# cvg/nice-slam

Measured on NVIDIA H100. Metric: rendered rays/sec, higher is better.
Workload: dtype f32

## Files before the change

nice_slam_b200/csrc/nsb_aux.cu:

```cuda
#include <cstdarg>
#include <cstdio>
#include <cstring>
#include <type_traits>
#include <cuda_fp16.h>
#include "nsb_common.cuh"
#include "nsb_seeds.cuh"
#include "nsb_geom.cuh"

namespace nsb {

static thread_local char g_err[512] = "";
void set_error(const char* fmt, ...) {
  va_list ap; va_start(ap, fmt); vsnprintf(g_err, sizeof(g_err), fmt, ap); va_end(ap);
}
int check_cuda(cudaError_t e, const char* what) {
  if (e == cudaSuccess) return NSB_OK;
  set_error("%s: %s", what, cudaGetErrorString(e));
  (void)cudaGetLastError();
  return NSB_ERR_CUDA;
}

struct PackArgs { nsb_decoder_params p[4]; float* packed[4]; float* flat[4]; int present[4]; };
__device__ __forceinline__ bool pk_mine(int& e) { return (e++ % (int)gridDim.y) == (int)blockIdx.y; }
constexpr int kPackSlices = 32;
// ... 56 lines not shown
    const float h = __uint_as_float(__float_as_uint(v) & 0xffffe000u);
    const int o = ((r >> 3) * (KW >> 2) + (k >> 2)) * 32 + (r & 7) * 4 + (k & 3);
    hi[o] = h; lo[o] = v - h;
  }
}
template <int LV>
__device__ void pack_operands_level(float* __restrict__ img , int& e) {
  using D = Dec<LV>;
  const float* W = img;
  constexpr int PH = D::PH;
  const int o_wh[5] = {0, D::o_W1, D::o_W2, D::o_W3H, D::o_W4};
  float* dst = img + op_fwd_offset(LV);
  if (pk_mine(e)) for (int i = threadIdx.x; i < kHdrFloats; i += blockDim.x) {
    float v = 0.0f;
    if (i < 160) v = W[D::o_b + i];
    else if (i < 320) v = D::XYZ ? W[D::o_bc + (i - 160)] : 0.0f;
    else if (i < 324) v = W[D::o_bo + (i - 320)];
    else if (i >= 336 && i < 464) v = W[D::o_WO + ((i - 336) >> 5) * PH + ((i - 336) & 31)];
    else if (i >= 464 && i < 464 + 3 * kEmbPad) v = D::XYZ ? W[D::o_B + (i - 464)] : 0.0f;
    dst[i] = v;
  }
  dst += kHdrFloats;
  if (D::XYZ)
    for (int h = 0; h < D::CD / 32; h++)
      emit_unit(dst, e, 160, 32, [&](int r, int k) { return W[D::o_WC + r * D::PC + 32 * h + k]; });
  for (int b = 0; b < op_nblk(LV); b++)
    emit_unit(dst, e, 64, 32, [&](int r, int k) { return W[(r < 32 ? D::o_W0 : D::o_W3E) + (r & 31) * D::PF + 32 * b + k]; });
  for (int i = 1; i < 5; i++) emit_unit(dst, e, 32, 32, [&](int r, int k) { return W[o_wh[i] + r * PH + k]; });
  dst = img + op_bwd_offset(LV);
  for (int i = 4; i >= 0; i--) {
    if (D::XYZ) emit_unit(dst, e, D::CD, 32, [&](int c, int k) { return W[D::o_WC + (i * 32 + k) * D::PC + c]; });
    if (i >= 1) emit_unit(dst, e, 32, 32, [&](int j, int k) { return W[o_wh[i] + k * PH + j]; });
    if (i == 3 || i == 0) emit_unit(dst, e, D::FIRSTP, 32, [&](int f, int k) { return W[(i == 0 ? D::o_W0 : D::o_W3E) + k * D::PF + f]; });
  }
}
template <int LV>
__device__ void pack_units_level(float* __restrict__ img, int& e) {
  using D = Dec<LV>;
  const float* W = img;
  constexpr int PH = D::PH;
  const int o_wh[5] = {0, D::o_W1, D::o_W2, D::o_W3H, D::o_W4};
  float* dst = img + op2_fwd_offset(LV);
  if (D::XYZ)
    for (int u = 0; u < D::CD / 8; u++)
      emit_unit(dst, e, 160, 8, [&](int r, int k) { return W[D::o_WC + r * D::PC + 8 * u + k]; });
  for (int b = 0; b < op_nblk(LV); b++)
    for (int h = 0; h < 2; h++)
      emit_unit(dst, e, 64, 16, [&](int r, int k) { return W[(r < 32 ? D::o_W0 : D::o_W3E) + (r & 31) * D::PF + 32 * b + 16 * h + k]; });
  for (int i = 1; i < 5; i++) emit_unit(dst, e, 32, 32, [&](int r, int k) { return W[o_wh[i] + r * PH + k]; });
  dst = img + op2_bwd_offset(LV);
  for (int i = 4; i >= 0; i--) {
    if (D::XYZ)
      for (int c2 = 0; c2 < D::CD / 32; c2++)
        emit_unit(dst, e, 32, 32, [&](int c, int k) { return W[D::o_WC + (i * 32 + k) * D::PC + 32 * c2 + c]; });
    if (i >= 1) emit_unit(dst, e, 32, 32, [&](int j, int k) { return W[o_wh[i] + k * PH + j]; });
    if (i == 3 || i == 0)
      for (int fb = 0; fb < D::FIRSTP / 32; fb++)
        emit_unit(dst, e, 32, 32, [&](int f, int k) { return W[(i == 0 ? D::o_W0 : D::o_W3E) + k * D::PF + 32 * fb + f]; });
  }
}
template <typename F>
__device__ __forceinline__ void emit_unit_h16(__half*& dst, int& e, int R, int KW, F&& get) {
  __half* hi = dst; __half* lo = dst + R * KW;
  dst += 2 * R * KW;
  if (!pk_mine(e)) return;
  for (int idx = threadIdx.x; idx < R * KW; idx += blockDim.x) {
    const int r = idx / KW, k = idx - r * KW;
    const float v = get(r, k);
    const __half h = __float2half_rn(v);
    const int o = ((r >> 3) * (KW >> 3) + (k >> 3)) * 64 + (r & 7) * 8 + (k & 7);
    hi[o] = h; lo[o] = __float2half_rn(v - __half2float(h));
  }
}
template <int LV>
__device__ void pack_units_h16_level(float* __restrict__ img, int& e) {
  using D = Dec<LV>;
  const float* W = img;
  constexpr int PH = D::PH;
  const int o_wh[5] = {0, D::o_W1, D::o_W2, D::o_W3H, D::o_W4};
  __half* dst = reinterpret_cast<__half*>(img + op3_fwd_offset(LV));
  if (D::XYZ)
    for (int u = 0; u < D::CD / 16; u++)
      emit_unit_h16(dst, e, 160, 16, [&](int r, int k) { return W[D::o_WC + r * D::PC + 16 * u + k]; });
  for (int b = 0; b < op_nblk(LV); b++)
    emit_unit_h16(dst, e, 64, 32, [&](int r, int k) { return W[(r < 32 ? D::o_W0 : D::o_W3E) + (r & 31) * D::PF + 32 * b + k]; });
  for (int i = 1; i < 5; i++) emit_unit_h16(dst, e, 32, 32, [&](int r, int k) { return W[o_wh[i] + r * PH + k]; });
}
__global__ void pack_operands_kernel(const __grid_constant__ PackArgs A) {
  const int lv = blockIdx.x;
  if (!A.present[lv]) return;
  int e = 0;
  switch (lv) {
    case 0: pack_operands_level<0>(A.packed[0], e); pack_units_level<0>(A.packed[0], e); pack_units_h16_level<0>(A.packed[0], e); break;
    case 1: pack_operands_level<1>(A.packed[1], e); pack_units_level<1>(A.packed[1], e); pack_units_h16_level<1>(A.packed[1], e); break;
    case 2: pack_operands_level<2>(A.packed[2], e); pack_units_level<2>(A.packed[2], e); pack_units_h16_level<2>(A.packed[2], e); break;
    default: pack_operands_level<3>(A.packed[3], e); pack_units_level<3>(A.packed[3], e); pack_units_h16_level<3>(A.packed[3], e); break;
  }
}

int launch_unpack_grads(float* const d_packed[4], float* const d_flat[4], cudaStream_t st) {
  PackArgs A; memset(&A, 0, sizeof(A));
  for (int l = 0; l < 4; l++) { A.packed[l] = d_packed[l]; A.flat[l] = d_flat[l]; A.present[l] = d_packed[l] != nullptr && d_flat[l] != nullptr; }
  pack_kernel<1><<<dim3(4, kPackSlices), 256, 0, st>>>(A);
  return check_cuda(cudaGetLastError(), "unpack_grads launch");
}

__global__ void batch_max_kernel(const float* __restrict__ gt, int n, float* __restrict__ out2, const PeerX px) {
  __shared__ float red[32];
  float m = -INFINITY;
  for (int i = threadIdx.x; i < n; i += blockDim.x) m = fmaxf(m, gt[i]);
  for (int o = 16; o > 0; o >>= 1) m = fmaxf(m, __shfl_xor_sync(0xffffffffu, m, o));
// ... 834 lines not shown
```

nice_slam_b200/csrc/nsb_common.cuh:

```cuda
#pragma once
#include <cuda_runtime.h>
#include <cuda_fp16.h>
#include <stdint.h>
#include "../../include/nice_slam_b200.h"

namespace nsb {

constexpr int kHid = 32;
constexpr int kEmb = 93;
constexpr int kEmbPad = 96;
constexpr int kChunk = 16;
constexpr int kRowF = 16;
constexpr int kMaxPtsPerBlock = 384;
constexpr int kMaxRaysPerBlock = 24;

__host__ __device__ inline size_t align16(size_t x) { return (x + 15) & ~size_t(15); }

template <int LV>
struct Dec {
  static constexpr bool XYZ = LV != 0;
  static constexpr int CD = LV == 2 ? 64 : 32;
  static constexpr int NO = LV == 3 ? 4 : 1;
  static constexpr int FIRST = XYZ ? kEmb : 32;
  static constexpr int FIRSTP = XYZ ? kEmbPad : 32;
  static constexpr int PF = FIRSTP + 4;
  static constexpr int PH = kHid + 4;
  static constexpr int PC = CD + 4;
  static constexpr int o_B = 0;
  static constexpr int o_W0 = XYZ ? 3 * kEmbPad : 0;
  static constexpr int o_W1 = o_W0 + 32 * PF;
  static constexpr int o_W2 = o_W1 + 32 * PH;
  static constexpr int o_W3E = o_W2 + 32 * PH;
  static constexpr int o_W3H = o_W3E + 32 * PF;
  static constexpr int o_W4 = o_W3H + 32 * PH;
  static constexpr int o_WC = o_W4 + 32 * PH;
  static constexpr int o_WO = o_WC + (XYZ ? 160 * PC : 0);
  static constexpr int o_b = o_WO + 4 * PH;
  static constexpr int o_bc = o_b + 160;
  static constexpr int o_bo = o_bc + (XYZ ? 160 : 0);
  static constexpr int TOTAL = o_bo + 4;
  static_assert(TOTAL % 4 == 0, "packed image must be a multiple of 16 bytes");
  static constexpr int ROWS_FWD = 32 + 64 + 64;
  static constexpr int ROWS_BWD = 32 + 64 + 160 + 32 + 32;
};

__host__ __device__ constexpr int packed_floats(int lv) {
  return lv == 0 ? Dec<0>::TOTAL : lv == 1 ? Dec<1>::TOTAL : lv == 2 ? Dec<2>::TOTAL : Dec<3>::TOTAL;
}
constexpr int kMaxPacked = Dec<2>::TOTAL;
constexpr int kRowsFwd = Dec<2>::ROWS_FWD;
constexpr int kRowsBwd = Dec<2>::ROWS_BWD;

constexpr int kHdrFloats = 768;
__host__ __device__ constexpr int op_cd(int lv) { return lv == 2 ? 64 : 32; }
__host__ __device__ constexpr int op_firstp(int lv) { return lv == 0 ? 32 : kEmbPad; }
__host__ __device__ constexpr int op_nblk(int lv) { return lv == 0 ? 1 : 3; }
constexpr int kFcChunk = 2 * 160 * 32, kL0Chunk = 2 * 64 * 32, kHChunk = 2 * 32 * 32;
__host__ __device__ constexpr int op_fc_floats(int lv) { return lv == 0 ? 0 : (op_cd(lv) / 32) * kFcChunk; }
__host__ __device__ constexpr int op_fwd_floats(int lv) { return kHdrFloats + op_fc_floats(lv) + op_nblk(lv) * kL0Chunk + 4 * kHChunk; }
__host__ __device__ constexpr int op_bwd_layer_floats(int lv, int i) {
  return (lv != 0 ? 2 * op_cd(lv) * 32 : 0) + (i >= 1 ? kHChunk : 0) + ((i == 3 || i == 0) ? 2 * op_firstp(lv) * 32 : 0);
}
__host__ __device__ constexpr int op_bwd_layer_offset(int lv, int i) {
  int off = 0;
  for (int j = 4; j > i; j--) off += op_bwd_layer_floats(lv, j);
  return off;
}
__host__ __device__ constexpr int op_bwd_floats(int lv) { return op_bwd_layer_offset(lv, -1); }
__host__ __device__ constexpr int op_fwd_offset(int lv) { return packed_floats(lv); }
__host__ __device__ constexpr int op_bwd_offset(int lv) { return packed_floats(lv) + op_fwd_floats(lv); }
__host__ __device__ constexpr int op2_fc_units(int lv) { return lv == 0 ? 0 : op_cd(lv) / 8; }
__host__ __device__ constexpr int op2_fwd_units(int lv) { return op2_fc_units(lv) + 2 * op_nblk(lv) + 4; }
__host__ __device__ constexpr int op2_fwd_floats(int lv) { return op2_fc_units(lv) * 2560 + (2 * op_nblk(lv) + 4) * 2048; }
__host__ __device__ constexpr int op2_bwd_layer_units(int lv, int i) {
  return (lv != 0 ? op_cd(lv) / 32 : 0) + (i >= 1 ? 1 : 0) + ((i == 3 || i == 0) ? op_firstp(lv) / 32 : 0);
}
__host__ __device__ constexpr int op2_bwd_units(int lv) {
  int n = 0;
  for (int i = 0; i < 5; i++) n += op2_bwd_layer_units(lv, i);
  return n;
}
__host__ __device__ constexpr int op2_bwd_floats(int lv) { return op2_bwd_units(lv) * 2048; }
__host__ __device__ constexpr int op2_fwd_offset(int lv) { return packed_floats(lv) + op_fwd_floats(lv) + op_bwd_floats(lv); }
__host__ __device__ constexpr int op2_bwd_offset(int lv) { return op2_fwd_offset(lv) + op2_fwd_floats(lv); }
__host__ __device__ constexpr int op3_fc_units(int lv) { return lv == 0 ? 0 : op_cd(lv) / 16; }
__host__ __device__ constexpr int op3_fwd_units(int lv) { return op3_fc_units(lv) + op_nblk(lv) + 4; }
__host__ __device__ constexpr int op3_fwd_floats(int lv) { return op3_fc_units(lv) * 2560 + op_nblk(lv) * 2048 + 4 * 1024; }
__host__ __device__ constexpr int op3_fwd_offset(int lv) { return op2_bwd_offset(lv) + op2_bwd_floats(lv); }
__host__ __device__ constexpr int packed_total_floats(int lv) { return op3_fwd_offset(lv) + op3_fwd_floats(lv); }
constexpr int kBwdStageFloats = op_bwd_layer_floats(2, 3);
static_assert(kBwdStageFloats == 12288, "backward stage size");

__host__ __device__ inline int dec_in(int lv, int i) {
  if (lv == 0) return i == 3 ? 64 : 32;
  return i == 0 ? kEmb : (i == 3 ? kEmb + kHid : kHid);
}
__host__ __device__ inline long long flat_offset(int lv, int kind, int layer) {
  const bool xyz = lv != 0;
  const int cd = lv == 2 ? 64 : 32, no = lv == 3 ? 4 : 1;
  long long off = 0;
  if (xyz) { if (kind == 0) return off; off += 3 * kEmb; }
  for (int i = 0; i < 5; i++) {
    if (kind == 1 && layer == i) return off; off += (long long)kHid * dec_in(lv, i);
    if (kind == 2 && layer == i) return off; off += kHid;
  }
  if (xyz) for (int i = 0; i < 5; i++) {
    if (kind == 3 && layer == i) return off; off += (long long)kHid * cd;
    if (kind == 4 && layer == i) return off; off += kHid;
  }
  if (kind == 5) return off; off += (long long)no * kHid;
  if (kind == 6) return off; off += no;
  return off;
}

__device__ __forceinline__ uint32_t smem_u32(const void* p) { return (uint32_t)__cvta_generic_to_shared(p); }

__device__ __forceinline__ void mbar_init(uint64_t* bar, uint32_t count) {
  asm volatile("mbarrier.init.shared::cta.b64 [%0], %1;" ::"r"(smem_u32(bar)), "r"(count) : "memory");
}
__device__ __forceinline__ void mbar_fence_init() { asm volatile("fence.mbarrier_init.release.cluster;" ::: "memory"); }
__device__ __forceinline__ void fence_proxy_async() { asm volatile("fence.proxy.async.shared::cta;" ::: "memory"); }
__device__ __forceinline__ void mbar_expect_tx(uint64_t* bar, uint32_t bytes) {
  asm volatile("mbarrier.arrive.expect_tx.shared::cta.b64 _, [%0], %1;" ::"r"(smem_u32(bar)), "r"(bytes) : "memory");
// ... 55 lines not shown
```

nice_slam_b200/csrc/nsb_tc.cuh:

```cuda
#pragma once

namespace nsb {
namespace tc {

#ifdef NSB_PHASE_TIMING
__device__ long long g_phase[64];
__device__ long long g_phase_last;
#define NSB_PH(id) do { if (blockIdx.x == 0 && threadIdx.x == 0) { const long long c_ = clock64(); ::nsb::tc::g_phase[id] += c_ - ::nsb::tc::g_phase_last; ::nsb::tc::g_phase_last = c_; } } while (0)
#define NSB_PH_RESET() do { if (blockIdx.x == 0 && threadIdx.x == 0) ::nsb::tc::g_phase_last = clock64(); } while (0)
#else
#define NSB_PH(id) do { } while (0)
#define NSB_PH_RESET() do { } while (0)
#endif

constexpr int TM = 128;
constexpr int kThreads = 512;
constexpr int kCG = kThreads / TM;
constexpr int kCW = 32 / kCG;
constexpr int kKQ = kCW / 4;

__device__ __forceinline__ float to_tf32(float x) { return __uint_as_float(__float_as_uint(x) & 0xffffe000u); }

__device__ __forceinline__ int canon_q(int r, int kq, int K) { return ((r >> 3) * (K >> 2) + kq) * 32 + (r & 7) * 4; }

// ... 10 lines not shown
  uint64_t d = 0;
  d |= (uint64_t)((smem_u32(smem) >> 4) & 0x3FFF);
  d |= (uint64_t)((lbo_bytes >> 4) & 0x3FFF) << 16;
  d |= (uint64_t)((sbo_bytes >> 4) & 0x3FFF) << 32;
  return d;
}

constexpr int kAccCols = 256;
constexpr int kAccSlotsPerSm = 4;
constexpr int kAccMaxSm = 144;
__device__ float g_acc_pool[(size_t)kAccMaxSm * kAccSlotsPerSm * kAccCols * TM];
__device__ int g_acc_lock[kAccMaxSm * kAccSlotsPerSm];
__shared__ float* s_acc;
__device__ __forceinline__ uint32_t acc_acquire() {
  uint32_t smid;
  asm volatile("mov.u32 %0, %%smid;" : "=r"(smid));
  if (smid >= (uint32_t)kAccMaxSm) __trap();
  const long long t0 = clock64();
  for (;;) {
    for (int k = 0; k < kAccSlotsPerSm; k++) {
      const int s = (int)smid * kAccSlotsPerSm + k;
      if (atomicCAS(&g_acc_lock[s], 0, 1) == 0) {
        __threadfence();
        s_acc = g_acc_pool + (size_t)s * kAccCols * TM;
        return (uint32_t)s;
      }
    }
    if (clock64() - t0 > 4000000000ll) __trap();
  }
}
__device__ __forceinline__ void acc_release(uint32_t slot) { __threadfence(); atomicExch(&g_acc_lock[slot], 0); }
__device__ __forceinline__ const float* acc_col(uint32_t taddr) { return s_acc + (size_t)(taddr & 0xffffu) * TM + (taddr >> 16) + (threadIdx.x & 31); }

__device__ __forceinline__ void wg_fence() { asm volatile("wgmma.fence.sync.aligned;" ::: "memory"); }
__device__ __forceinline__ void wg_commit_wait() {
  asm volatile("wgmma.commit_group.sync.aligned;" ::: "memory");
  asm volatile("wgmma.wait_group.sync.aligned 0;" ::: "memory");
}
__device__ __forceinline__ void wg_commit() { asm volatile("wgmma.commit_group.sync.aligned;" ::: "memory"); }
__device__ __forceinline__ void wg_wait0() { asm volatile("wgmma.wait_group.sync.aligned 0;" ::: "memory"); }
template <int N>
__device__ __forceinline__ void wg_wait() { asm volatile("wgmma.wait_group.sync.aligned %0;" ::"n"(N) : "memory"); }
__device__ __forceinline__ void fence_acc(float (&d)[16]) {
#pragma unroll
  for (int e = 0; e < 16; e++) asm volatile("" : "+f"(d[e])::"memory");
}
#define NSB_WG_D16 "+f"(d[0]), "+f"(d[1]), "+f"(d[2]), "+f"(d[3]), "+f"(d[4]), "+f"(d[5]), "+f"(d[6]), "+f"(d[7]), \
                   "+f"(d[8]), "+f"(d[9]), "+f"(d[10]), "+f"(d[11]), "+f"(d[12]), "+f"(d[13]), "+f"(d[14]), "+f"(d[15])
__device__ __forceinline__ void wgmma_tf32_n32(float (&d)[16], uint64_t da, uint64_t db) {
  asm volatile("{\n\t.reg .pred p;\n\tsetp.ne.b32 p, 1, 0;\n\t"
               "wgmma.mma_async.sync.aligned.m64n32k8.f32.tf32.tf32 "
               "{%0,%1,%2,%3,%4,%5,%6,%7,%8,%9,%10,%11,%12,%13,%14,%15}, %16, %17, p, 1, 1;\n\t}"
               : NSB_WG_D16 : "l"(da), "l"(db));
}
__device__ __forceinline__ void wgmma_f16_n32(float (&d)[16], uint64_t da, uint64_t db) {
  asm volatile("{\n\t.reg .pred p;\n\tsetp.ne.b32 p, 1, 0;\n\t"
               "wgmma.mma_async.sync.aligned.m64n32k16.f32.f16.f16 "
               "{%0,%1,%2,%3,%4,%5,%6,%7,%8,%9,%10,%11,%12,%13,%14,%15}, %16, %17, p, 1, 1, 0, 0;\n\t}"
               : NSB_WG_D16 : "l"(da), "l"(db));
}
#define NSB_WG_D32 "+f"(d0[0]), "+f"(d0[1]), "+f"(d0[2]), "+f"(d0[3]), "+f"(d0[4]), "+f"(d0[5]), "+f"(d0[6]), "+f"(d0[7]), \
                   "+f"(d0[8]), "+f"(d0[9]), "+f"(d0[10]), "+f"(d0[11]), "+f"(d0[12]), "+f"(d0[13]), "+f"(d0[14]), "+f"(d0[15]), \
                   "+f"(d1[0]), "+f"(d1[1]), "+f"(d1[2]), "+f"(d1[3]), "+f"(d1[4]), "+f"(d1[5]), "+f"(d1[6]), "+f"(d1[7]), \
                   "+f"(d1[8]), "+f"(d1[9]), "+f"(d1[10]), "+f"(d1[11]), "+f"(d1[12]), "+f"(d1[13]), "+f"(d1[14]), "+f"(d1[15])
#define NSB_WG_R32 "{%0,%1,%2,%3,%4,%5,%6,%7,%8,%9,%10,%11,%12,%13,%14,%15,%16,%17,%18,%19,%20,%21,%22,%23,%24,%25,%26,%27,%28,%29,%30,%31}"
__device__ __forceinline__ void wgmma_tf32_n64(float (&d0)[16], float (&d1)[16], uint64_t da, uint64_t db) {
  asm volatile("{\n\t.reg .pred p;\n\tsetp.ne.b32 p, 1, 0;\n\t"
               "wgmma.mma_async.sync.aligned.m64n64k8.f32.tf32.tf32 " NSB_WG_R32 ", %32, %33, p, 1, 1;\n\t}"
               : NSB_WG_D32 : "l"(da), "l"(db));
}
__device__ __forceinline__ void wgmma_f16_n64(float (&d0)[16], float (&d1)[16], uint64_t da, uint64_t db) {
  asm volatile("{\n\t.reg .pred p;\n\tsetp.ne.b32 p, 1, 0;\n\t"
               "wgmma.mma_async.sync.aligned.m64n64k16.f32.f16.f16 " NSB_WG_R32 ", %32, %33, p, 1, 1, 0, 0;\n\t}"
               : NSB_WG_D32 : "l"(da), "l"(db));
}
__device__ __forceinline__ void frag_rc(int e, int& r, int& c) {
  const int l = threadIdx.x & 31, w = (threadIdx.x >> 5) & 3;
  r = 16 * w + (l >> 2) + 8 * ((e >> 1) & 1);
  c = 8 * (e >> 2) + 2 * (l & 3) + (e & 1);
}

template <bool H16>
__device__ __forceinline__ void wg_mma(uint32_t dcol, uint64_t ah, uint64_t al, uint32_t sboA, uint64_t bh, uint64_t bl, uint32_t sboB,
                                       int N, int ksteps, uint32_t acc) {
  const int wg = threadIdx.x >> 7, npairs = blockDim.x >> 8;
  const int rbase = 64 * (wg & 1);
  const uint64_t aoff = (uint64_t)((8u * sboA * (uint32_t)(wg & 1)) >> 4);
  for (int c = wg >> 1; c < (N >> 5); c += npairs) {
    float* base = s_acc + (size_t)(dcol + 32 * c) * TM + rbase;
    float d[16];
#pragma unroll
    for (int e = 0; e < 16; e++) { int r, cc; frag_rc(e, r, cc); d[e] = acc ? base[cc * TM + r] : 0.0f; }
    const uint64_t boff = (uint64_t)((4u * sboB * (uint32_t)c) >> 4);
    wg_fence();
#pragma unroll 1
    for (int ks = 0; ks < ksteps; ks++) {
      const uint64_t o = 16u * (uint64_t)ks;
      if (H16) {
        wgmma_f16_n32(d, al + aoff + o, bh + boff + o); wgmma_f16_n32(d, ah + aoff + o, bl + boff + o); wgmma_f16_n32(d, ah + aoff + o, bh + boff + o);
      } else {
        wgmma_tf32_n32(d, al + aoff + o, bh + boff + o); wgmma_tf32_n32(d, ah + aoff + o, bl + boff + o); wgmma_tf32_n32(d, ah + aoff + o, bh + boff + o);
      }
    }
    wg_commit_wait();
#pragma unroll
    for (int e = 0; e < 16; e++) { int r, cc; frag_rc(e, r, cc); base[cc * TM + r] = d[e]; }
// ... 381 lines not shown
```

nice_slam_b200/csrc/nsb_tile.cuh:

```cuda
#pragma once

namespace nsb {
namespace tl {

using tc::TM;
constexpr int kThreads = 256;
constexpr int kEpiThreads = kThreads;
constexpr int kCG = 2, kCW = 16, kKQ = 4;
constexpr int kSlots = 4;
constexpr int kSlotFloatsFwd = 2560;
constexpr int kSlotFloatsBwd = 2048;
constexpr int kABufFloats = 2 * TM * 32;
constexpr int kMaxTileRays = 18;
constexpr int kMinSamples = 8;
constexpr long long kWaitCycles = 4000000000ll;

enum { B_FULL = 0, B_EMPTY = 4, B_HDR = 8, B_AREADY = 10, B_DONE = 12, kNumBars = 14 };

__device__ __forceinline__ bool mbar_try(uint64_t* bar, uint32_t parity) {
  uint32_t ok;
  asm volatile("{\n\t.reg .pred p;\n\tmbarrier.try_wait.parity.shared::cta.b64 p, [%1], %2;\n\tselp.b32 %0, 1, 0, p;\n\t}"
               : "=r"(ok) : "r"(smem_u32(bar)), "r"(parity) : "memory");
  return ok != 0;
}
// ... 153 lines not shown
  r.ah = tc::make_desc(a + (ka0 / kcm) * 32, 128u, sbo_a) + (uint64_t)((8u * sbo_a * g) >> 4);
  r.bh = tc::make_desc(b, 128u, sbo_b) + (uint64_t)((4u * sbo_b * (uint32_t)c) >> 4);
  r.al = r.ah + (uint64_t)((TM * 32 * esz) >> 4); r.bl = r.bh + (uint64_t)((N * KB * esz) >> 4);
  return r;
}
template <bool H16, int ksteps>
__device__ __forceinline__ void mma_rows(float (&d)[16], const float* a, int ka0, const float* b, int N, int KB, int c) {
  const RowsDesc r = rows_desc<H16>(a, ka0, b, N, KB, c);
#pragma unroll
  for (int ks = 0; ks < ksteps; ks++) {
    const uint64_t o = 16u * (uint64_t)ks;
    if (H16) { tc::wgmma_f16_n32(d, r.al + o, r.bh + o); tc::wgmma_f16_n32(d, r.ah + o, r.bl + o); tc::wgmma_f16_n32(d, r.ah + o, r.bh + o); }
    else { tc::wgmma_tf32_n32(d, r.al + o, r.bh + o); tc::wgmma_tf32_n32(d, r.ah + o, r.bl + o); tc::wgmma_tf32_n32(d, r.ah + o, r.bh + o); }
  }
}
template <bool H16, int ksteps>
__device__ __forceinline__ void mma_rows64(float (&d0)[16], float (&d1)[16], const float* a, int ka0, const float* b, int N, int KB, int c) {
  const RowsDesc r = rows_desc<H16>(a, ka0, b, N, KB, c);
#pragma unroll
  for (int ks = 0; ks < ksteps; ks++) {
    const uint64_t o = 16u * (uint64_t)ks;
    if (H16) { tc::wgmma_f16_n64(d0, d1, r.al + o, r.bh + o); tc::wgmma_f16_n64(d0, d1, r.ah + o, r.bl + o); tc::wgmma_f16_n64(d0, d1, r.ah + o, r.bh + o); }
    else { tc::wgmma_tf32_n64(d0, d1, r.al + o, r.bh + o); tc::wgmma_tf32_n64(d0, d1, r.ah + o, r.bl + o); tc::wgmma_tf32_n64(d0, d1, r.ah + o, r.bh + o); }
  }
}
__device__ __forceinline__ void arrive_units(const TileSmem& t, uint32_t first, uint32_t count, uint64_t* done = nullptr) {
  if ((threadIdx.x & 127) == 0) {
    for (uint32_t k = 0; k < count; k++) mbar_arrive(t.bars + B_EMPTY + ((first + k) & (kSlots - 1)));
    if (done != nullptr) mbar_arrive(done);
  }
}
__device__ __forceinline__ void release_units(Issuer& I, const TileSmem& t, uint32_t count, uint64_t* done = nullptr) {
  arrive_units(t, I.issued, count, done);
  I.issued += count;
}
__device__ __forceinline__ void wg_bar_sync() {
  if (threadIdx.x >> 7) asm volatile("bar.sync 2, 128;" ::: "memory");
  else asm volatile("bar.sync 1, 128;" ::: "memory");
}
__device__ __forceinline__ void zero16(float (&d)[16]) {
#pragma unroll
  for (int e = 0; e < 16; e++) d[e] = 0.0f;
}
__device__ __forceinline__ void zero16_opaque(float (&d)[16]) {
#pragma unroll
  for (int e = 0; e < 16; e++) asm volatile("mov.b32 %0, 0;" : "=f"(d[e])::"memory");
}
__device__ __forceinline__ void put2(float* hi, int r, int c, float a, float b) {
  float* hp = hi + tc::canon_q(r, c >> 2, 32) + (c & 3);
  const float h0 = tc::to_tf32(a), h1 = tc::to_tf32(b);
  *reinterpret_cast<float2*>(hp) = make_float2(h0, h1);
  *reinterpret_cast<float2*>(hp + TM * 32) = make_float2(a - h0, b - h1);
}

__device__ __forceinline__ void publish(const TileSmem& t, int b) {
  fence_proxy_async();
  __syncwarp();
  if ((threadIdx.x & 31) == 0) mbar_arrive(t.bars + B_AREADY + b);
}
__device__ __forceinline__ void wait_group(const TileSmem& t, uint32_t m) {
  mbar_wait_b(t.bars + B_DONE + (m & 1u), (m >> 1) & 1u);
}

struct GatherPass {
  float4 v[8];
  float w[8];
  int src_lane;
};
template <bool FAST>
__device__ __forceinline__ void gather_issue(const nsb_grid& g, const float xn[3], int it, int lane, GatherPass& gp) {
  const int q = lane & 7;
  gp.src_lane = it * 4 + (lane >> 3);
  float x[3];
  x[0] = __shfl_sync(0xffffffffu, xn[0], gp.src_lane); x[1] = __shfl_sync(0xffffffffu, xn[1], gp.src_lane); x[2] = __shfl_sync(0xffffffffu, xn[2], gp.src_lane);
  const Tri t = make_tri(x, g.W, g.H, g.D);
  const long long ox[2] = {(long long)t.i0[0] * g.stride_w, (long long)min(t.i0[0] + 1, g.W - 1) * g.stride_w};
  const long long oy[2] = {(long long)t.i0[1] * g.stride_h, (long long)min(t.i0[1] + 1, g.H - 1) * g.stride_h};
  const long long oz[2] = {(long long)t.i0[2] * g.stride_d, (long long)min(t.i0[2] + 1, g.D - 1) * g.stride_d};
#pragma unroll
  for (int k = 0; k < 8; k++) gp.v[k] = grid_load4(g, oz[k >> 2] + oy[(k >> 1) & 1] + ox[k & 1], 4 * q, FAST);
  const float wxy[4] = {__fmul_rn(t.w0[0], t.w0[1]), __fmul_rn(t.w1[0], t.w0[1]), __fmul_rn(t.w0[0], t.w1[1]), __fmul_rn(t.w1[0], t.w1[1])};
#pragma unroll
  for (int k = 0; k < 8; k++) gp.w[k] = __fmul_rn(wxy[k & 3], (k & 4) ? t.w1[2] : t.w0[2]);
}
template <bool H16 = false>
__device__ __forceinline__ void gather_consume(float* c_hi, float* c_lo, int qd, int lane, const GatherPass& gp) {
  float4 acc = make_float4(0.f, 0.f, 0.f, 0.f);
#pragma unroll
  for (int k = 0; k < 8; k++) {
    const float w = gp.w[k];
    acc.x = fmaf(gp.v[k].x, w, acc.x); acc.y = fmaf(gp.v[k].y, w, acc.y); acc.z = fmaf(gp.v[k].z, w, acc.z); acc.w = fmaf(gp.v[k].w, w, acc.w);
  }
  if (H16) put4_h(c_hi, qd * 32 + gp.src_lane, lane & 7, acc);
  else tc::put4(c_hi, c_lo, qd * 32 + gp.src_lane, lane & 7, 32, acc);
}
template <bool FAST, bool H16 = false>
__device__ __forceinline__ void gather_tile_t(const nsb_grid& g, float* c_hi, const float xn[3], int warp, int lane) {
  float* c_lo = c_hi + TM * 32;
  const int qd = warp & 3, it0 = (warp >> 2) * 4;
  if (FAST) {
    GatherPass A, B;
    gather_issue<true>(g, xn, it0, lane, A);
    gather_issue<true>(g, xn, it0 + 1, lane, B);
    gather_consume<H16>(c_hi, c_lo, qd, lane, A);
    gather_issue<true>(g, xn, it0 + 2, lane, A);
    gather_consume<H16>(c_hi, c_lo, qd, lane, B);
// ... 317 lines not shown
    }
  }
  __syncthreads();
}
__device__ __forceinline__ float warp_colsum16(const float (&v)[kCW], int lane) {
  float a[8];
#pragma unroll
  for (int j = 0; j < 8; j++) { const float give = (lane & 16) ? v[j] : v[j + 8], keep = (lane & 16) ? v[j + 8] : v[j]; a[j] = keep + __shfl_xor_sync(0xffffffffu, give, 16); }
  float b[4];
#pragma unroll
  for (int j = 0; j < 4; j++) { const float give = (lane & 8) ? a[j] : a[j + 4], keep = (lane & 8) ? a[j + 4] : a[j]; b[j] = keep + __shfl_xor_sync(0xffffffffu, give, 8); }
  float c[2];
#pragma unroll
  for (int j = 0; j < 2; j++) { const float give = (lane & 4) ? b[j] : b[j + 2], keep = (lane & 4) ? b[j + 2] : b[j]; c[j] = keep + __shfl_xor_sync(0xffffffffu, give, 4); }
  const float give = (lane & 2) ? c[0] : c[1], keep = (lane & 2) ? c[1] : c[0];
  float d = keep + __shfl_xor_sync(0xffffffffu, give, 2);
  d += __shfl_xor_sync(0xffffffffu, d, 1);
  return d;
}
__device__ __forceinline__ int colsum_col(int lane) { return ((lane >> 4) & 1) * 8 + ((lane >> 3) & 1) * 4 + ((lane >> 2) & 1) * 2 + ((lane >> 1) & 1); }
__device__ __forceinline__ float frag_colsum(const float (&v)[16], int lane) {
  float a[8];
#pragma unroll
  for (int j = 0; j < 8; j++) a[j] = v[4 * (j >> 1) + (j & 1)] + v[4 * (j >> 1) + (j & 1) + 2];
  float b[4];
#pragma unroll
  for (int j = 0; j < 4; j++) { const float give = (lane & 16) ? a[j] : a[j + 4], keep = (lane & 16) ? a[j + 4] : a[j]; b[j] = keep + __shfl_xor_sync(0xffffffffu, give, 16); }
  float c[2];
#pragma unroll
  for (int j = 0; j < 2; j++) { const float give = (lane & 8) ? b[j] : b[j + 2], keep = (lane & 8) ? b[j + 2] : b[j]; c[j] = keep + __shfl_xor_sync(0xffffffffu, give, 8); }
  const float give = (lane & 4) ? c[0] : c[1], keep = (lane & 4) ? c[1] : c[0];
  return keep + __shfl_xor_sync(0xffffffffu, give, 4);
}
__device__ __forceinline__ int frag_colsum_col(int lane) {
  const int j = ((lane >> 4) & 1) * 4 + ((lane >> 3) & 1) * 2 + ((lane >> 2) & 1);
  return 8 * (j >> 1) + 2 * (lane & 3) + (j & 1);
}

struct BwdExtra {
  double dp[TM * 3];
  double z[TM];
  float gocc[TM];
  float wgt[TM];
  float gc[kMaxTileRays * 3];
};
__device__ __forceinline__ void bwd_gout(const BwdExtra& X, int lv, int r, int npts, int off0, int S, float (&go)[4]) {
  go[0] = go[1] = go[2] = go[3] = 0.0f;
  if (r >= npts) return;
  if (lv == 3) { const float w = X.wgt[r]; const float* gc = X.gc + 3 * ((off0 + r) / S); go[0] = w * gc[0]; go[1] = w * gc[1]; go[2] = w * gc[2]; }
  else go[0] = X.gocc[r];
}

template <bool DC, int NDF, bool L0>
__device__ __forceinline__ void issue_bwd_layer_t(Issuer& I, const TileSmem& t, int ndc, float (&d1)[16], float (&dc)[16], float (&fa)[16]) {
  constexpr int ND1 = L0 ? 0 : 1, FMAX = L0 ? 2 : 1;
  constexpr int kWaves = NDF > FMAX ? (NDF + FMAX - 1) / FMAX : 1;
#pragma unroll
  for (int wave = 0; wave < kWaves; wave++) {
    const int f0 = wave * FMAX;
    const int nf = NDF - f0 < FMAX ? NDF - f0 : FMAX;
    const int k = wave == 0 ? ndc + ND1 : 0;
    const int nu = k + nf;
#pragma unroll 1
    for (int u = 0; u < nu; u++) issuer_unit(I, t, u);
    if (nf > 0) { if (L0) ld_frag(d2_frag(f0), fa); else zero16_opaque(fa); }
    if (nf > 1) ld_frag(d2_frag(f0 + 1), d1);
    if (wave == 0 && ND1) zero16_opaque(d1);
    tc::wg_fence();
    if (wave == 0) {
      if (DC) mma_rows<false, 4>(dc, t.a[0], 0, issued_unit(I, t, 0), 32, 32, 0);
      if (ND1) mma_rows<false, 4>(d1, t.a[1], 0, issued_unit(I, t, ndc), 32, 32, 0);
    }
    if (nf > 0) mma_rows<false, 4>(fa, t.a[1], 0, issued_unit(I, t, k), 32, 32, 0);
    if (nf > 1) mma_rows<false, 4>(d1, t.a[1], 0, issued_unit(I, t, k + 1), 32, 32, 0);
    tc::wg_commit(); tc::wg_wait0();
    tc::fence_acc(dc); tc::fence_acc(d1); tc::fence_acc(fa);
    if (nf > 0) st_frag(d2_frag(f0), fa);
    if (nf > 1) st_frag(d2_frag(f0 + 1), d1);
    release_units(I, t, nu);
  }
}
template <bool XYZ>
__device__ __forceinline__ void issue_bwd_layer_x(Issuer& I, const TileSmem& t, int ndc, int i, float (&d1)[16], float (&dc)[16], float (&fa)[16]) {
  constexpr int NDF = op_firstp(XYZ ? 1 : 0) / 32;
  if (XYZ && i == 4) zero16_opaque(dc);
  if (i == 3) issue_bwd_layer_t<XYZ, NDF, false>(I, t, ndc, d1, dc, fa);
  else if (i == 0) issue_bwd_layer_t<XYZ, NDF, true>(I, t, ndc, d1, dc, fa);
  else issue_bwd_layer_t<XYZ, 0, false>(I, t, ndc, d1, dc, fa);
}
__device__ __forceinline__ void issue_bwd_layer(Issuer& I, const TileSmem& t, int lv, int i, float (&d1)[16], float (&dc)[16], float (&fa)[16]) {
  if (lv != 0) issue_bwd_layer_x<true>(I, t, op_cd(lv) / 32, i, d1, dc, fa);
  else issue_bwd_layer_x<false>(I, t, 0, i, d1, dc, fa);
}

enum { kWgNone = 0, kWgXyz = 1, kWgCoarse = 2 };
__device__ __forceinline__ int bwd_dpe_off(int r) { return (r >> 6) * (64 * 32) + (r & 63) * 4; }
template <int WG>
__device__ __forceinline__ void epi_backward(const KParams& P, const TileSmem& t, Issuer& I, const BwdExtra& X, int lv, const PointGeom& G, int hb, uint32_t hdr_parity,
                                             const uint32_t* __restrict__ masks, int npts, int off0, long long gp0, WgSmem* w = nullptr, const float* acts_row = nullptr) {
  const int row = threadIdx.x & (TM - 1), cg = threadIdx.x >> 7, warp = threadIdx.x >> 5;
  const int lane = threadIdx.x & 31, q = lane & 3;
  const int r0 = 64 * (threadIdx.x >> 7) + 16 * (warp & 3) + (lane >> 2);
  const int S = P.S;
  constexpr bool kWg = WG != kWgNone;
  constexpr int PH = Dec<3>::PH, PF = WG == kWgCoarse ? Dec<0>::PF : Dec<3>::PF;
  const WgDec DW = WG == kWgCoarse ? wg_dec<0>() : lv == 2 ? wg_dec<2>() : wg_dec<3>();
  float creg[kCW], cmid[kCW];
  const bool xyz = WG == kWgCoarse ? false : lv != 0;
  const float* hdr = t.hdr + hb * kHdrFloats;
  uint32_t m01 = 0, m23 = 0, m4 = 0;
  {
    const uint32_t* w0 = masks + (size_t)(r0 < npts ? r0 : npts - 1) * 15;
    const uint32_t* w1 = masks + (size_t)(r0 + 8 < npts ? r0 + 8 : npts - 1) * 15;
#pragma unroll
    for (int i = 0; i < 5; i++) {
      const uint32_t v = ((w0[i] >> (2 * q)) & 0x03030303u) | (((w1[i] >> (2 * q)) & 0x03030303u) << 2);
      if (i == 4) m4 = v; else if (i & 2) m23 |= v << (4 * (i & 1)); else m01 |= v << (4 * (i & 1));
    }
  }
  mbar_wait_b(t.bars + B_HDR + hb, hdr_parity);
  float d1[16], dc[16], fa[16];
  {
    float go0[4], go1[4];
    bwd_gout(X, lv, r0, npts, off0, S, go0); bwd_gout(X, lv, r0 + 8, npts, off0, S, go1);
#pragma unroll
    for (int e = 0; e < 16; e++) {
      float v = 0.0f;
#pragma unroll
      for (int o = 0; o < 4; o++) v = fmaf(hdr[336 + o * 32 + 8 * (e >> 2) + 2 * q + (e & 1)], (e & 2) ? go1[o] : go0[o], v);
      d1[e] = v;
    }
  }
  if constexpr (kWg) {
    float g_out[4];
    bwd_gout(X, lv, row, npts, off0, S, g_out);
    gather_tile_kt(P.in.grid[lv], w->b, kWgBLo, WG == kWgCoarse ? G.xnc : G.xn, warp, lane);
    __syncthreads();
    get_kt16(w->b, kWgBLo, row, cg, creg);
    __syncthreads();
    if (lv == 2) {
      gather_tile_kt(P.in.grid[NSB_MIDDLE], w->b, kWgBLo, G.xn, warp, lane);
      __syncthreads();
      get_kt16(w->b, kWgBLo, row, cg, cmid);
      __syncthreads();
    }
    float go[kCW];
#pragma unroll
    for (int j = 0; j < kCW; j++) go[j] = (cg == 0 && j < 4) ? g_out[j] : 0.0f;
    put_kt16(w->du, kWgALo, row, cg, go);
    float h4[kCW];
#pragma unroll
    for (int k = 0; k < kKQ; k++) {
      const float4 v = acts_row != nullptr ? __ldcg(reinterpret_cast<const float4*>(acts_row + 4 * 32 + 4 * k)) : make_float4(0.f, 0.f, 0.f, 0.f);
      h4[4 * k] = v.x; h4[4 * k + 1] = v.y; h4[4 * k + 2] = v.z; h4[4 * k + 3] = v.w;
    }
    put_kt16(w->b, kWgBLo, row, cg, h4);
    wg_group(*w, 0, w->dpk + DW.o_WO, PH, DW.no);
    if (cg == 0) {
      const float sb = warp_colsum16(go, lane);
      const int col = colsum_col(lane);
      if ((lane & 1) == 0 && col < DW.no) atomicAdd(w->dpk + DW.o_bo + col, sb);
    }
  }
#pragma unroll 1
  for (int i = 4; i >= 0; i--) {
    const uint32_t m = (i == 4 ? m4 : (i & 2) ? m23 : m01) >> (4 * (i & 1));
    float du[16];
#pragma unroll
    for (int e = 0; e < 16; e++) du[e] = (m >> (8 * (e >> 2) + 2 * ((e >> 1) & 1) + (e & 1))) & 1u ? d1[e] : 0.0f;
#pragma unroll
    for (int e = 0; e < 16; e += 2) {
      const int r = r0 + 8 * ((e >> 1) & 1), c = 8 * (e >> 2) + 2 * q;
      if (xyz) put2(t.a[0], r, c, d1[e], d1[e + 1]);
      put2(t.a[1], r, c, du[e], du[e + 1]);
    }
    if constexpr (kWg) {
#pragma unroll
      for (int e = 0; e < 16; e++) {
        const int r = r0 + 8 * ((e >> 1) & 1), c = 8 * (e >> 2) + 2 * q + (e & 1);
        put_kt1(w->du, kWgALo, c, r, du[e]);
        if constexpr (WG != kWgCoarse) put_kt1(w->g, kWgALo, c, r, d1[e]);
      }
      const float sb = frag_colsum(du, lane);
      float sc = 0.0f;
      if constexpr (WG != kWgCoarse) sc = frag_colsum(d1, lane);
      const int col = frag_colsum_col(lane);
      atomicAdd(w->dpk + DW.o_b + 32 * i + col, sb);
      if constexpr (WG != kWgCoarse) atomicAdd(w->dpk + DW.o_bc + 32 * i + col, sc);
    }
    fence_proxy_async();
    wg_bar_sync();
    NSB_PH(22);
    issue_bwd_layer(I, t, WG == kWgCoarse ? 0 : lv, i, d1, dc, fa);
    if (threadIdx.x == 0) loader_top_up(I.L, t, I.issued);
    NSB_PH(23);
    if constexpr (kWg) {
      if (i >= 1) {
        float xr[kCW];
#pragma unroll
        for (int k = 0; k < kKQ; k++) {
          const float4 v = acts_row != nullptr ? __ldcg(reinterpret_cast<const float4*>(acts_row + (i - 1) * 32 + 4 * k)) : make_float4(0.f, 0.f, 0.f, 0.f);
          xr[4 * k] = v.x; xr[4 * k + 1] = v.y; xr[4 * k + 2] = v.z; xr[4 * k + 3] = v.w;
        }
        put_kt16(w->b, kWgBLo, row, cg, xr);
        const int o_wh = i == 1 ? DW.o_W1 : i == 2 ? DW.o_W2 : i == 3 ? DW.o_W3H : DW.o_W4;
        wg_group(*w, 0, w->dpk + o_wh, PH, 32);
      }
      if constexpr (WG != kWgCoarse) {
        put_kt16(w->b, kWgBLo, row, cg, creg);
        wg_group(*w, 1, w->dpk + DW.o_WC + 32 * i * DW.PC, DW.PC, 32);
        if (lv == 2) {
          put_kt16(w->b, kWgBLo, row, cg, cmid);
          wg_group(*w, 1, w->dpk + DW.o_WC + 32 * i * DW.PC + 32, DW.PC, 32);
        }
      }
      if (i == 3 || i == 0) {
        if constexpr (WG != kWgCoarse) {
          const float* B = hdr + 464;
          for (int blk = 0; blk < 3; blk++) {
            float e[kCW];
#pragma unroll
            for (int j = 0; j < kCW; j++) {
              const int f = 32 * blk + kCW * cg + j;
              float x = G.pf[0] * B[f]; x = fmaf(G.pf[1], B[kEmbPad + f], x); x = fmaf(G.pf[2], B[2 * kEmbPad + f], x);
              e[j] = f < kEmb ? __sinf(reduce_2pi(x)) : 0.0f;
            }
            put_kt16(w->b, kWgBLo, row, cg, e);
            wg_group(*w, 0, w->dpk + (i == 0 ? DW.o_W0 : DW.o_W3E) + 32 * blk, PF, 32);
          }
        } else {
          put_kt16(w->b, kWgBLo, row, cg, creg);
          wg_group(*w, 0, w->dpk + (i == 0 ? DW.o_W0 : DW.o_W3E), PF, 32);
        }
      }
      NSB_PH(24);
    }
  }
  if (!xyz) ld_frag(d2_frag(0), dc);
#pragma unroll
  for (int e = 0; e < 16; e += 2) {
    const int r = r0 + 8 * ((e >> 1) & 1), c = 8 * (e >> 2) + 2 * q;
    *reinterpret_cast<float2*>(t.a[0] + r * 32 + c) = make_float2(dc[e], dc[e + 1]);
  }
  float dpe0[3] = {0.0f, 0.0f, 0.0f}, dpe1[3] = {0.0f, 0.0f, 0.0f};
  if (xyz) {
    const float* B = hdr + 464;
// ... 374 lines not shown
```

Measured before the change: 1.254 million.

## Feed backward du operand to wgmma from registers instead of shared memory

The backward layer now builds a split-TF32 register A-fragment from the masked gradient and issues wgmma with register-sourced A (RS form), so it no longer writes du to shared memory or waits on a fence and barrier before those MMAs. Backward weight units are packed with a permuted K order (op2_bwd_k) to match the register fragment layout. The xyz dc path still stages through shared memory, with the barrier moved so it overlaps the already-committed RS MMAs. This raises register pressure and carries correctness risk from the K permutation.

```diff
diff --git a/nice_slam_b200/csrc/nsb_aux.cu b/nice_slam_b200/csrc/nsb_aux.cu
--- a/nice_slam_b200/csrc/nsb_aux.cu
+++ b/nice_slam_b200/csrc/nsb_aux.cu
@@ -132,11 +132,11 @@
   for (int i = 4; i >= 0; i--) {
     if (D::XYZ)
       for (int c2 = 0; c2 < D::CD / 32; c2++)
-        emit_unit(dst, e, 32, 32, [&](int c, int k) { return W[D::o_WC + (i * 32 + k) * D::PC + 32 * c2 + c]; });
-    if (i >= 1) emit_unit(dst, e, 32, 32, [&](int j, int k) { return W[o_wh[i] + k * PH + j]; });
+        emit_unit(dst, e, 32, 32, [&](int c, int k) { return W[D::o_WC + (i * 32 + op2_bwd_k(k)) * D::PC + 32 * c2 + c]; });
+    if (i >= 1) emit_unit(dst, e, 32, 32, [&](int j, int k) { return W[o_wh[i] + op2_bwd_k(k) * PH + j]; });
     if (i == 3 || i == 0)
       for (int fb = 0; fb < D::FIRSTP / 32; fb++)
-        emit_unit(dst, e, 32, 32, [&](int f, int k) { return W[(i == 0 ? D::o_W0 : D::o_W3E) + k * D::PF + 32 * fb + f]; });
+        emit_unit(dst, e, 32, 32, [&](int f, int k) { return W[(i == 0 ? D::o_W0 : D::o_W3E) + op2_bwd_k(k) * D::PF + 32 * fb + f]; });
   }
 }
 template <typename F>
diff --git a/nice_slam_b200/csrc/nsb_common.cuh b/nice_slam_b200/csrc/nsb_common.cuh
--- a/nice_slam_b200/csrc/nsb_common.cuh
+++ b/nice_slam_b200/csrc/nsb_common.cuh
@@ -69,6 +69,7 @@
 __host__ __device__ constexpr int op_bwd_floats(int lv) { return op_bwd_layer_offset(lv, -1); }
 __host__ __device__ constexpr int op_fwd_offset(int lv) { return packed_floats(lv); }
 __host__ __device__ constexpr int op_bwd_offset(int lv) { return packed_floats(lv) + op_fwd_floats(lv); }
+__host__ __device__ constexpr int op2_bwd_k(int p) { return (p & ~7) | ((p & 7) < 4 ? 2 * (p & 3) : 2 * (p & 3) + 1); }
 __host__ __device__ constexpr int op2_fc_units(int lv) { return lv == 0 ? 0 : op_cd(lv) / 8; }
 __host__ __device__ constexpr int op2_fwd_units(int lv) { return op2_fc_units(lv) + 2 * op_nblk(lv) + 4; }
 __host__ __device__ constexpr int op2_fwd_floats(int lv) { return op2_fc_units(lv) * 2560 + (2 * op_nblk(lv) + 4) * 2048; }
diff --git a/nice_slam_b200/csrc/nsb_tc.cuh b/nice_slam_b200/csrc/nsb_tc.cuh
--- a/nice_slam_b200/csrc/nsb_tc.cuh
+++ b/nice_slam_b200/csrc/nsb_tc.cuh
@@ -86,6 +86,12 @@
                "wgmma.mma_async.sync.aligned.m64n32k8.f32.tf32.tf32 "
                "{%0,%1,%2,%3,%4,%5,%6,%7,%8,%9,%10,%11,%12,%13,%14,%15}, %16, %17, p, 1, 1;\n\t}"
                : NSB_WG_D16 : "l"(da), "l"(db));
+}
+__device__ __forceinline__ void wgmma_tf32_n32_rs(float (&d)[16], const uint32_t (&a)[4], uint64_t db) {
+  asm volatile("{\n\t.reg .pred p;\n\tsetp.ne.b32 p, 1, 0;\n\t"
+               "wgmma.mma_async.sync.aligned.m64n32k8.f32.tf32.tf32 "
+               "{%0,%1,%2,%3,%4,%5,%6,%7,%8,%9,%10,%11,%12,%13,%14,%15}, {%16,%17,%18,%19}, %20, p, 1, 1;\n\t}"
+               : NSB_WG_D16 : "r"(a[0]), "r"(a[1]), "r"(a[2]), "r"(a[3]), "l"(db));
 }
 __device__ __forceinline__ void wgmma_f16_n32(float (&d)[16], uint64_t da, uint64_t db) {
   asm volatile("{\n\t.reg .pred p;\n\tsetp.ne.b32 p, 1, 0;\n\t"
diff --git a/nice_slam_b200/csrc/nsb_tile.cuh b/nice_slam_b200/csrc/nsb_tile.cuh
--- a/nice_slam_b200/csrc/nsb_tile.cuh
+++ b/nice_slam_b200/csrc/nsb_tile.cuh
@@ -229,6 +229,39 @@
   *reinterpret_cast<float2*>(hp) = make_float2(h0, h1);
   *reinterpret_cast<float2*>(hp + TM * 32) = make_float2(a - h0, b - h1);
 }
+__device__ __forceinline__ void put2_bwd(float* hi, int r, int c, float a, float b) {
+  float* hp = hi + tc::canon_q(r, (c >> 3) * 2, 32) + ((c & 7) >> 1);
+  const float h0 = tc::to_tf32(a), h1 = tc::to_tf32(b);
+  hp[0] = h0; hp[32] = h1;
+  hp[TM * 32] = a - h0; hp[TM * 32 + 32] = b - h1;
+}
+struct FragA { uint32_t h[4][4], l[4][4]; };
+__device__ __forceinline__ void frag_a(const float (&d)[16], FragA& a) {
+#pragma unroll
+  for (int j = 0; j < 4; j++) {
+#pragma unroll
+    for (int v = 0; v < 4; v++) {
+      const float x = d[4 * j + 2 * (v & 1) + (v >> 1)], h = tc::to_tf32(x);
+      a.h[j][v] = __float_as_uint(h); a.l[j][v] = __float_as_uint(x - h);
+    }
+  }
+}
+__device__ __forceinline__ void fence_a(FragA& a) {
+#pragma unroll
+  for (int j = 0; j < 4; j++)
+#pragma unroll
+    for (int v = 0; v < 4; v++) asm volatile("" : "+r"(a.h[j][v]), "+r"(a.l[j][v])::"memory");
+}
+template <int ksteps>
+__device__ __forceinline__ void mma_rows_rs(float (&d)[16], const FragA& a, const float* b, int N, int KB, int c) {
+  const uint32_t sbo_b = (uint32_t)(KB / 4) * 128u;
+  const uint64_t bh = tc::make_desc(b, 128u, sbo_b) + (uint64_t)((4u * sbo_b * (uint32_t)c) >> 4), bl = bh + (uint64_t)((N * KB * 4) >> 4);
+#pragma unroll
+  for (int ks = 0; ks < ksteps; ks++) {
+    const uint64_t o = 16u * (uint64_t)ks;
+    tc::wgmma_tf32_n32_rs(d, a.l[ks], bh + o); tc::wgmma_tf32_n32_rs(d, a.h[ks], bl + o); tc::wgmma_tf32_n32_rs(d, a.h[ks], bh + o);
+  }
+}
 
 __device__ __forceinline__ void publish(const TileSmem& t, int b) {
   fence_proxy_async();
@@ -652,7 +685,7 @@
 }
 
 template <bool DC, int NDF, bool L0>
-__device__ __forceinline__ void issue_bwd_layer_t(Issuer& I, const TileSmem& t, int ndc, float (&d1)[16], float (&dc)[16], float (&fa)[16]) {
+__device__ __forceinline__ void issue_bwd_layer_t(Issuer& I, const TileSmem& t, int ndc, float (&d1)[16], float (&dc)[16], float (&fa)[16], FragA& du) {
   constexpr int ND1 = L0 ? 0 : 1, FMAX = L0 ? 2 : 1;
   constexpr int kWaves = NDF > FMAX ? (NDF + FMAX - 1) / FMAX : 1;
 #pragma unroll
@@ -666,14 +699,19 @@
     if (nf > 0) { if (L0) ld_frag(d2_frag(f0), fa); else zero16_opaque(fa); }
     if (nf > 1) ld_frag(d2_frag(f0 + 1), d1);
     if (wave == 0 && ND1) zero16_opaque(d1);
+    fence_a(du);
     tc::wg_fence();
-    if (wave == 0) {
-      if (DC) mma_rows<false, 4>(dc, t.a[0], 0, issued_unit(I, t, 0), 32, 32, 0);
-      if (ND1) mma_rows<false, 4>(d1, t.a[1], 0, issued_unit(I, t, ndc), 32, 32, 0);
-    }
-    if (nf > 0) mma_rows<false, 4>(fa, t.a[1], 0, issued_unit(I, t, k), 32, 32, 0);
-    if (nf > 1) mma_rows<false, 4>(d1, t.a[1], 0, issued_unit(I, t, k + 1), 32, 32, 0);
-    tc::wg_commit(); tc::wg_wait0();
+    if (wave == 0 && ND1) mma_rows_rs<4>(d1, du, issued_unit(I, t, ndc), 32, 32, 0);
+    if (nf > 0) mma_rows_rs<4>(fa, du, issued_unit(I, t, k), 32, 32, 0);
+    if (nf > 1) mma_rows_rs<4>(d1, du, issued_unit(I, t, k + 1), 32, 32, 0);
+    tc::wg_commit();
+    if (wave == 0 && DC) {
+      fence_proxy_async();
+      wg_bar_sync();
+      mma_rows<false, 4>(dc, t.a[0], 0, issued_unit(I, t, 0), 32, 32, 0);
+      tc::wg_commit();
+    }
+    tc::wg_wait0();
     tc::fence_acc(dc); tc::fence_acc(d1); tc::fence_acc(fa);
     if (nf > 0) st_frag(d2_frag(f0), fa);
     if (nf > 1) st_frag(d2_frag(f0 + 1), d1);
@@ -681,16 +719,16 @@
   }
 }
 template <bool XYZ>
-__device__ __forceinline__ void issue_bwd_layer_x(Issuer& I, const TileSmem& t, int ndc, int i, float (&d1)[16], float (&dc)[16], float (&fa)[16]) {
+__device__ __forceinline__ void issue_bwd_layer_x(Issuer& I, const TileSmem& t, int ndc, int i, float (&d1)[16], float (&dc)[16], float (&fa)[16], FragA& du) {
   constexpr int NDF = op_firstp(XYZ ? 1 : 0) / 32;
   if (XYZ && i == 4) zero16_opaque(dc);
-  if (i == 3) issue_bwd_layer_t<XYZ, NDF, false>(I, t, ndc, d1, dc, fa);
-  else if (i == 0) issue_bwd_layer_t<XYZ, NDF, true>(I, t, ndc, d1, dc, fa);
-  else issue_bwd_layer_t<XYZ, 0, false>(I, t, ndc, d1, dc, fa);
-}
-__device__ __forceinline__ void issue_bwd_layer(Issuer& I, const TileSmem& t, int lv, int i, float (&d1)[16], float (&dc)[16], float (&fa)[16]) {
-  if (lv != 0) issue_bwd_layer_x<true>(I, t, op_cd(lv) / 32, i, d1, dc, fa);
-  else issue_bwd_layer_x<false>(I, t, 0, i, d1, dc, fa);
+  if (i == 3) issue_bwd_layer_t<XYZ, NDF, false>(I, t, ndc, d1, dc, fa, du);
+  else if (i == 0) issue_bwd_layer_t<XYZ, NDF, true>(I, t, ndc, d1, dc, fa, du);
+  else issue_bwd_layer_t<XYZ, 0, false>(I, t, ndc, d1, dc, fa, du);
+}
+__device__ __forceinline__ void issue_bwd_layer(Issuer& I, const TileSmem& t, int lv, int i, float (&d1)[16], float (&dc)[16], float (&fa)[16], FragA& du) {
+  if (lv != 0) issue_bwd_layer_x<true>(I, t, op_cd(lv) / 32, i, d1, dc, fa, du);
+  else issue_bwd_layer_x<false>(I, t, 0, i, d1, dc, fa, du);
 }
 
 enum { kWgNone = 0, kWgXyz = 1, kWgCoarse = 2 };
@@ -768,11 +806,11 @@
     float du[16];
 #pragma unroll
     for (int e = 0; e < 16; e++) du[e] = (m >> (8 * (e >> 2) + 2 * ((e >> 1) & 1) + (e & 1))) & 1u ? d1[e] : 0.0f;
-#pragma unroll
-    for (int e = 0; e < 16; e += 2) {
-      const int r = r0 + 8 * ((e >> 1) & 1), c = 8 * (e >> 2) + 2 * q;
-      if (xyz) put2(t.a[0], r, c, d1[e], d1[e + 1]);
-      put2(t.a[1], r, c, du[e], du[e + 1]);
+    FragA du_a;
+    frag_a(du, du_a);
+    if (xyz) {
+#pragma unroll
+      for (int e = 0; e < 16; e += 2) put2_bwd(t.a[0], r0 + 8 * ((e >> 1) & 1), 8 * (e >> 2) + 2 * q, d1[e], d1[e + 1]);
     }
     if constexpr (kWg) {
 #pragma unroll
@@ -788,10 +826,8 @@
       atomicAdd(w->dpk + DW.o_b + 32 * i + col, sb);
       if constexpr (WG != kWgCoarse) atomicAdd(w->dpk + DW.o_bc + 32 * i + col, sc);
     }
-    fence_proxy_async();
-    wg_bar_sync();
     NSB_PH(22);
-    issue_bwd_layer(I, t, WG == kWgCoarse ? 0 : lv, i, d1, dc, fa);
+    issue_bwd_layer(I, t, WG == kWgCoarse ? 0 : lv, i, d1, dc, fa, du_a);
     if (threadIdx.x == 0) loader_top_up(I.L, t, I.issued);
     NSB_PH(23);
     if constexpr (kWg) {
```

Measured after the change: 1.288 million (median of 6 runs). +2.7%, better.
